# lcicek/Critic-VAE

Hardware: AMD Instinct MI355X
Metric: VAE train-step images/sec on 64x64x3 frames (higher is better)
Workload: dtype f32

## Files before the change

### critic-vae_amd/csrc/api.hip

```cpp
#include "common.h"
#include "../../include/cvae.h"
#include <stdarg.h>
#include <stdio.h>
#include <stdlib.h>
#include <string.h>
#include <cmath>
#include <string>
#include <vector>

static thread_local char g_err[512] = "";
void cvae_set_error(const char* fmt, ...) {
    va_list ap;
    va_start(ap, fmt);
    vsnprintf(g_err, sizeof(g_err), fmt, ap);
    va_end(ap);
}

static constexpr int PROBE_IDS = 32, PROBE_CAP = 128;
struct ProbeSlot { hipEvent_t e0[PROBE_CAP], e1[PROBE_CAP]; int n = 0; bool made = false; };
struct ProbeState { uint32_t mask = 0; ProbeSlot slot[PROBE_IDS]; };
static thread_local ProbeSlot* g_probe_cur = nullptr;
void cvae_probe_begin(hipStream_t st) {
    ProbeSlot* p = g_probe_cur;
    if (p && p->n < PROBE_CAP) (void)hipEventRecord(p->e0[p->n], st);
}
void cvae_probe_end(hipStream_t st) {
    ProbeSlot* p = g_probe_cur;
    if (p && p->n < PROBE_CAP) { (void)hipEventRecord(p->e1[p->n], st); p->n++; }
}

int cvae_num_cus() {
    constexpr int NCACHE = 64;
    static std::atomic<int> cached[NCACHE];
    int dev = 0;
    hipError_t e = hipGetDevice(&dev);
    if (e != hipSuccess) { cvae_set_error("cvae_num_cus: hipGetDevice failed (%s); assuming 256 compute units", hipGetErrorString(e)); return 256; }
    const bool cacheable = dev >= 0 && dev < NCACHE;
    int n = cacheable ? cached[dev].load(std::memory_order_relaxed) : 0;
    if (n > 0) return n;
    e = hipDeviceGetAttribute(&n, hipDeviceAttributeMultiprocessorCount, dev);
    if (e != hipSuccess || n <= 0) {
        cvae_set_error("cvae_num_cus: compute-unit query failed on device %d (%s); assuming 256", dev, hipGetErrorString(e));
        return 256;
    }
    if (cacheable) cached[dev].store(n, std::memory_order_relaxed);
    return n;
}

int persistent_grid(int wgs_per_cu, int num_items) {
    static const int maxwg = [] { const char* e = getenv("CVAE_PERSIST_MAXWG"); const int n = e ? atoi(e) : 0; return n > 0 ? n : 0; }();
    int G = wgs_per_cu * cvae_num_cus();
    if (maxwg > 0 && G > maxwg) G = maxwg;
    G -= G % 8;
    if (G < 8) G = 8;
    return G < num_items ? G : num_items;
}
extern "C" int32_t cvae_conv_route(int32_t precision, int32_t width, int32_t layer, int32_t dgrad, int64_t batch) {
    if ((width != 64 && width != 128) || layer < 0 || layer > 3 || precision < 0 || precision > 3 || batch < 1 || batch > 0x7fffffffLL) return CVAE_EINVAL;
    if (layer == 0 && (precision != 1 || dgrad != 0)) return CVAE_EINVAL;
    return conv_route(precision, layer, width, dgrad != 0, batch).family;
}

struct ParamEntry { std::string name; int64_t offset, numel; };

struct WsLayout {
    int64_t y[4], a[4], coef[4], bnpart[4];
    int64_t zcat, h, o[4];
    int64_t dout4, d_o[4], d_h, d_zcat, d_a[4], d_y[4];
    int64_t wc[3];
    int64_t xp;
    int64_t wpack;
    int64_t ms, scratch_w, scratch, total;
};

struct cvae_handle_s {
    cvae_config cfg;
    std::vector<ParamEntry> params;
    int64_t param_total;
    int K;
    int enc_w[4], enc_b[4], enc_g[4], enc_be[4], fc_w, fc_b, dec_w[5], dec_b[5], di_w, di_b;
    hipStream_t side = nullptr;
    hipEvent_t ev_ready[8] = {}, ev_side = nullptr;
    bool streams_ready = false;
    bool e1_two_pass = false;
    const void* xp_ws = nullptr;
    int xp_B = 0;
    bool fuse_e1 = true;
    ProbeState probe;
};

struct ProbeArm {
    ProbeArm(cvae_handle_s* h, int kind, int layer) {
        const int id = kind * 9 + layer;
        g_probe_cur = (h->probe.mask >> id) & 1u ? &h->probe.slot[id] : nullptr;
    }
    ~ProbeArm() { g_probe_cur = nullptr; }
};

static int ensure_streams(cvae_handle_s* h) {
    if (h->streams_ready) return 0;
    int lo = 0, hi = 0;
    hipError_t e = hipDeviceGetStreamPriorityRange(&lo, &hi);
    if (e == hipSuccess) e = hipStreamCreateWithPriority(&h->side, hipStreamNonBlocking, lo);
    for (int i = 0; i < 8 && e == hipSuccess; ++i) e = hipEventCreateWithFlags(&h->ev_ready[i], hipEventDisableTiming);
    if (e == hipSuccess) e = hipEventCreateWithFlags(&h->ev_side, hipEventDisableTiming);
    if (e != hipSuccess) { cvae_set_error("side stream setup failed: %s", hipGetErrorString(e)); return (int)e; }
    h->streams_ready = true;
    return 0;
}

static int layer_h(const cvae_handle_s* h, int layer) { return kLayers[layer].h * (h->cfg.width / 64); }

static WsLayout carve(const cvae_handle_s* h, int B) {
    WsLayout w{};
    const int W = h->cfg.width;
    int64_t off = 0;
    auto take = [&](int64_t n) { int64_t o = off; off += align_up(n, 64); return o; };
    const bool b16 = h->cfg.precision == 1;
    auto act = [&](int64_t elems) { return take(b16 ? (elems + 1) / 2 : elems); };
    for (int l = 0; l < 4; ++l) {
        const int64_t H = layer_h(h, l), C = kLayers[l].cout;
        w.y[l] = act(B * H * H * C);
        w.a[l] = act(B * (H / 2) * (H / 2) * C);
        w.coef[l] = take(C * 4);
        w.bnpart[l] = take((int64_t)2 * bn_num_tiles(l, W, B) * C);
        w.d_y[l] = (l == 0 && h->fuse_e1) ? -1 : act(B * H * H * C);
        w.d_a[l] = act(B * (H / 2) * (H / 2) * C);
    }
    w.zcat = take((int64_t)B * 33);
    w.d_zcat = take((int64_t)B * 33);
    w.h = act((int64_t)B * h->K);
    w.d_h = act((int64_t)B * h->K);
    for (int i = 0; i < 4; ++i) {
        const int64_t H = layer_h(h, 4 + i), C = kLayers[4 + i].cout;
        w.o[i] = act(B * H * H * C);
        w.d_o[i] = act(B * H * H * C);
    }
    w.dout4 = take(b16 ? 0 : (int64_t)B * 3 * W * W);
    for (int i = 0; i < 3; ++i) w.wc[i] = take(conv_up_wc_floats(5 + i));
    w.xp = take(b16 ? (int64_t)B * W * W * 2 : 0);
    w.wpack = take(h->cfg.precision != 0 ? conv_bf16_pack_floats(h->cfg.precision >= 2 ? 3 : 1) : 0);
    w.ms = take(msssim_ws_floats(W, B));
    int64_t sc = 0, scw = 0;
    auto mx = [&](int64_t v) { if (v > sc) sc = v; };
    for (int l = 1; l <= 4; ++l) { if (wgrad_ws_floats(l, W, B) > scw) scw = wgrad_ws_floats(l, W, B);
        if (h->cfg.precision == 1 && conv_bf16_supported(l, W) && wgrad_bf16_ws_floats(l, W, B) > scw) scw = wgrad_bf16_ws_floats(l, W, B);
        if (h->cfg.precision >= 2 && conv_bf16_supported(l, W) && wgrad_split_ws_floats(l, W, B) > scw) scw = wgrad_split_ws_floats(l, W, B);
        mx(conv_fwd_ws_floats(l, W, B)); mx(conv_dgrad_ws_floats(l, W, B)); }
    for (int l = 5; l <= 7; ++l) { if (conv_up_wgrad_ws_floats(l, W, B) > scw) scw = conv_up_wgrad_ws_floats(l, W, B); mx(conv_up_ws_floats(l, W, B)); }
    if (e1_wgrad_ws_floats(W, B) > scw) scw = e1_wgrad_ws_floats(W, B);
    w.scratch_w = take(scw);
    mx(scw + 36 * 128 * 64);
    mx(d4_bwd_ws_floats(W, B));
    for (int l = 0; l < 4; ++l) { mx(bn_bwd_ws_floats(l, W, B)); mx(bn_fwd_ws_floats(l, W)); }
    mx(fc_ws_floats(W, B));
    mx(colsum_ws_floats(0, 256));
    w.scratch = take(sc);
    w.total = off;
    return w;
}

static void add_param(cvae_handle_s* h, int* idx, const char* name, int64_t numel) {
    *idx = (int)h->params.size();
    h->params.push_back(ParamEntry{name, h->param_total, numel});
    h->param_total += align_up(numel, 64);
}

extern "C" {

const char* cvae_version(void) { return "critic-vae_amd 0.3 (gfx950; fp32 MFMA, bf16 MFMA with bf16 storage)"; }
const char* cvae_last_error(void) { return g_err; }

int cvae_create(const cvae_config* cfg, cvae_handle* out) {
    if (!cfg || !out) { cvae_set_error("cvae_create: null argument"); return CVAE_EINVAL; }
    if (cfg->width != 64 && cfg->width != 128) { cvae_set_error("cvae_create: width %d not supported (64 or 128)", cfg->width); return CVAE_EUNSUPPORTED; }
    if (cfg->precision < 0 || cfg->precision > 3) { cvae_set_error("cvae_create: precision %d not supported (0 = fp32, 1 = bf16 MFMA, 2 = fp32 emulated by 3-way bf16 splits)", cfg->precision); return CVAE_EUNSUPPORTED; }
    cvae_handle_s* h = new cvae_handle_s();
    h->cfg = *cfg;
    { const char* e = getenv("CVAE_FUSE_E1"); h->fuse_e1 = !(e && e[0] == '0'); }
    { const char* e = getenv("CVAE_E1_TWO_PASS"); h->e1_two_pass = cfg->precision == 1 && !(e && e[0] == '0'); }
    h->param_total = 0;
    h->K = 256 * (cfg->width / 16) * (cfg->width / 16);
    char nm[64];
    for (int l = 0; l < 4; ++l) {
        snprintf(nm, sizeof nm, "enc%d.w", l); add_param(h, &h->enc_w[l], nm, (int64_t)25 * kLayers[l].cin * kLayers[l].cout);
        snprintf(nm, sizeof nm, "enc%d.b", l); add_param(h, &h->enc_b[l], nm, kLayers[l].cout);
        snprintf(nm, sizeof nm, "enc%d.gamma", l); add_param(h, &h->enc_g[l], nm, kLayers[l].cout);
        snprintf(nm, sizeof nm, "enc%d.beta", l); add_param(h, &h->enc_be[l], nm, kLayers[l].cout);
    }
    add_param(h, &h->fc_w, "fc.w", (int64_t)h->K * 64);
    add_param(h, &h->fc_b, "fc.b", 64);
    for (int i = 0; i < 5; ++i) {
        snprintf(nm, sizeof nm, "dec%d.w", i); add_param(h, &h->dec_w[i], nm, (int64_t)25 * kLayers[4 + i].cin * kLayers[4 + i].cout);
        snprintf(nm, sizeof nm, "dec%d.b", i); add_param(h, &h->dec_b[i], nm, kLayers[4 + i].cout);
    }
    add_param(h, &h->di_w, "decin.w", (int64_t)33 * h->K);
    add_param(h, &h->di_b, "decin.b", h->K);
    *out = h;
    return CVAE_OK;
}

void cvae_destroy(cvae_handle h) {
    if (!h) return;
    if (h->streams_ready) {
        for (int i = 0; i < 8; ++i) (void)hipEventDestroy(h->ev_ready[i]);
        (void)hipEventDestroy(h->ev_side);
        (void)hipStreamDestroy(h->side);
    }
    delete h;
}

int64_t cvae_param_total(cvae_handle h) { return h->param_total; }
int32_t cvae_param_count(cvae_handle h) { return (int32_t)h->params.size(); }
// ... 452 lines not shown
```

### critic-vae_amd/csrc/common.h

```cpp
#pragma once
#include <hip/hip_runtime.h>
#include <stdint.h>
#include <stddef.h>
#include <atomic>

typedef float f32x16 __attribute__((ext_vector_type(16)));
typedef float f32x4 __attribute__((ext_vector_type(4)));
typedef __bf16 bf16x8 __attribute__((ext_vector_type(8)));

typedef __bf16 bf16x4 __attribute__((ext_vector_type(4)));

template <typename AT> struct Act;
template <> struct Act<float> {
    static constexpr bool BF16 = false;
    static __device__ __forceinline__ float ld(const float* p, size_t i) { return p[i]; }
    static __device__ __forceinline__ void st(float* p, size_t i, float v) { p[i] = v; }
    static __device__ __forceinline__ f32x4 ld4(const float* p, size_t i) { return *reinterpret_cast<const f32x4*>(p + i); }
    static __device__ __forceinline__ void st4(float* p, size_t i, f32x4 v) { *reinterpret_cast<f32x4*>(p + i) = v; }
};
template <> struct Act<__bf16> {
    static constexpr bool BF16 = true;
    static __device__ __forceinline__ float ld(const float* p, size_t i) { return (float)reinterpret_cast<const __bf16*>(p)[i]; }
    static __device__ __forceinline__ void st(float* p, size_t i, float v) { reinterpret_cast<__bf16*>(p)[i] = (__bf16)v; }
    static __device__ __forceinline__ f32x4 ld4(const float* p, size_t i) {
        const bf16x4 v = *reinterpret_cast<const bf16x4*>(reinterpret_cast<const __bf16*>(p) + i);
        return f32x4{(float)v[0], (float)v[1], (float)v[2], (float)v[3]};
    }
    static __device__ __forceinline__ void st4(float* p, size_t i, f32x4 v) {
        bf16x4 o;
        o[0] = (__bf16)v[0]; o[1] = (__bf16)v[1]; o[2] = (__bf16)v[2]; o[3] = (__bf16)v[3];
        *reinterpret_cast<bf16x4*>(reinterpret_cast<__bf16*>(p) + i) = o;
    }
    static __device__ __forceinline__ bf16x4 ld4raw(const float* p, size_t i) { return *reinterpret_cast<const bf16x4*>(reinterpret_cast<const __bf16*>(p) + i); }
    static __device__ __forceinline__ bf16x8 ld8(const float* p, size_t i) { return *reinterpret_cast<const bf16x8*>(reinterpret_cast<const __bf16*>(p) + i); }
    static __device__ __forceinline__ void st8(float* p, size_t i, bf16x8 v) { *reinterpret_cast<bf16x8*>(reinterpret_cast<__bf16*>(p) + i) = v; }
};

typedef short short4v __attribute__((ext_vector_type(4)));
typedef short short8v __attribute__((ext_vector_type(8)));
__device__ __forceinline__ bf16x8 tr_frag(const __bf16* p0, const __bf16* p1) {
    const short4v lo = __builtin_amdgcn_ds_read_tr16_b64_v4i16((__attribute__((address_space(3))) short4v*)p0);
    const short4v hi = __builtin_amdgcn_ds_read_tr16_b64_v4i16((__attribute__((address_space(3))) short4v*)p1);
    const short8v v = __builtin_shufflevector(lo, hi, 0, 1, 2, 3, 4, 5, 6, 7);
    return __builtin_bit_cast(bf16x8, v);
}

#define CVAE_LATENT 32
#define CVAE_ZCAT 33

struct LayerDesc { int cin, cout, h, up; };
static constexpr LayerDesc kLayers[9] = {
    {3, 32, 64, 0}, {32, 64, 32, 0}, {64, 128, 16, 0}, {128, 256, 8, 0},
    {256, 128, 4, 0}, {128, 64, 8, 1}, {64, 32, 16, 1}, {32, 32, 32, 1}, {32, 3, 64, 1}};

template <int H>
struct Tile {
    static constexpr int TW = H < 32 ? H : 32;
    static constexpr int TH = (128 / TW) < H ? (128 / TW) : H;
    static constexpr int IMGS = 128 / (TW * TH);
    static constexpr int HTW = TW + 4, HTH = TH + 4;
    static constexpr int HPI = HTW * HTH;
    static constexpr int HP = IMGS * HPI;
    static constexpr int PS = ((HP + 5) / 8) * 8 + 2;
    static constexpr int TILES_X = H / TW, TILES_Y = H / TH;
    static constexpr int TILES_PER_IMG = TILES_X * TILES_Y;
    static_assert(TW * TH * IMGS == 128, "tile must hold 128 pixels");
};

__host__ __device__ inline int cdiv(int a, int b) { return (a + b - 1) / b; }

__device__ __forceinline__ void vm_drained() { __builtin_amdgcn_s_waitcnt(0x0F70); }

__device__ __forceinline__ int xcd_tile(int x, int G) { return (G & 7) ? x : (x & 7) * (G >> 3) + (x >> 3); }
inline int64_t align_up(int64_t v, int64_t a) { return (v + a - 1) / a * a; }

__device__ __forceinline__ float wave_sum(float v) {
#pragma unroll
    for (int o = 32; o > 0; o >>= 1) v += __shfl_xor(v, o, 64);
    return v;
}
__device__ __forceinline__ double wave_sum_d(double v) {
#pragma unroll
    for (int o = 32; o > 0; o >>= 1) v += __shfl_xor(v, o, 64);
    return v;
}

__device__ __forceinline__ bool wg_arrive_last(unsigned* counter, unsigned total, unsigned* lds_word) {
    asm volatile("s_waitcnt vmcnt(0)" ::: "memory");
    __syncthreads();
    if (threadIdx.x == 0) {
        __builtin_amdgcn_fence(__ATOMIC_RELEASE, "agent");
        asm volatile("s_waitcnt vmcnt(0)" ::: "memory");
        const unsigned t = __hip_atomic_fetch_add(counter, 1u, __ATOMIC_RELAXED, __HIP_MEMORY_SCOPE_AGENT);
        const bool last = t == total - 1;
        if (last) {
            __hip_atomic_store(counter, 0u, __ATOMIC_RELAXED, __HIP_MEMORY_SCOPE_AGENT);
            __builtin_amdgcn_fence(__ATOMIC_ACQUIRE, "agent");
            asm volatile("s_waitcnt vmcnt(0)" ::: "memory");
        }
        *lds_word = last ? 1u : 0u;
    }
    __syncthreads();
    return *lds_word != 0u;
}

void cvae_probe_begin(hipStream_t st);
void cvae_probe_end(hipStream_t st);

void cvae_set_error(const char* fmt, ...);
#define CVAE_CHECK_LAUNCH()                                                        \
    do {                                                                           \
        hipError_t e_ = hipGetLastError();                                         \
        if (e_ != hipSuccess) {                                                    \
            cvae_set_error("%s:%d launch failed: %s", __FILE__, __LINE__,          \
                           hipGetErrorString(e_));                                 \
            return (int)e_;                                                        \
        }                                                                          \
    } while (0)

struct DeviceOnce { std::atomic<uint64_t> mask{0}; };
inline int cvae_grant_lds(DeviceOnce& once, const void* kernel, int bytes) {
    int dev = 0;
    hipError_t e = hipGetDevice(&dev);
    const uint64_t bit = 1ull << (dev & 63);
    if (e == hipSuccess && (once.mask.load(std::memory_order_acquire) & bit)) return 0;
    if (e == hipSuccess) e = hipFuncSetAttribute(kernel, hipFuncAttributeMaxDynamicSharedMemorySize, bytes);
    if (e != hipSuccess) { cvae_set_error("dynamic LDS opt-in (%d bytes) failed: %s", bytes, hipGetErrorString(e)); return (int)e; }
    once.mask.fetch_or(bit, std::memory_order_release);
    return 0;
}

int cvae_num_cus();
int persistent_grid(int wgs_per_cu, int num_items);

enum ConvFamily { CONV_PER_TILE = 0, CONV_PS = 1, CONV_BIG = 2, E1_PACKED_FRAME = 1 };
struct ConvRoute {
    ConvFamily family;
    int tilesPerPartial;
};
ConvRoute conv_route(int precision, int layer, int width, bool dgrad, int64_t B);

int launch_conv_fwd(int layer, int width, int B, const float* in, const float* w, const float* bias,
                    float* out, float* bnpart, float* ws, hipStream_t st);
int64_t conv_fwd_ws_floats(int layer, int width, int B);
int launch_conv_dgrad(int layer, int width, int B, const float* dout, const float* w,
                      const float* mask_src, float* din, float* ws, hipStream_t st);
int64_t conv_dgrad_ws_floats(int layer, int width, int B);
bool conv_bf16_supported(int layer, int width);
int64_t conv_bf16_pack_floats(int ns);
int launch_pack_w_bf16(const float* const w[4], float* packed, int ns, hipStream_t st);
int launch_conv_fwd_bf16(int layer, int width, int ns, int B, const float* in, const float* packed, const float* bias, float* out,
                         float* bnpart, float* ws, hipStream_t st, int* tilesPerPartial = nullptr);
int launch_conv_dgrad_bf16(int layer, int width, int ns, int B, const float* dout, const float* packed, float* din, float* ws, hipStream_t st);
int launch_pack_up_bf16(const float* const wc[3], float* packed, int ns, hipStream_t st);
int launch_conv_up_fwd_bf16(int layer, int width, int ns, int B, const float* in, const float* packed, const float* bias, float* out, hipStream_t st);
int launch_conv_up_dgrad_bf16(int layer, int width, int ns, int B, const float* dout, const float* packed, const float* aux, float* din, hipStream_t st);
int64_t wgrad_bf16_ws_floats(int layer, int width, int B);
int launch_conv_wgrad_bf16(int layer, int width, int B, const float* in, const float* dout, float* dw, float* dbias, float* ws, hipStream_t st);
bool conv_wgrad_split_supported(int products);
int64_t wgrad_split_ws_floats(int layer, int width, int B);
int launch_conv_wgrad_split(int layer, int width, int products, int B, const float* in, const float* dout, float* dw, float* dbias,
                            float* ws, hipStream_t st);
int launch_splitk_bias_relu(const float* slab, const float* bias, float* out, int64_t slice, int KS, int C, hipStream_t st, bool out_bf16 = false);
int64_t wgrad_ws_floats(int layer, int width, int B);
int launch_conv_wgrad(int layer, int width, int B, const float* in, const float* dout, float* dw,
                      float* dbias, float* ws, hipStream_t st);
int launch_reduce_slabs(const float* slab, float* dst, int64_t n, int S, int64_t stride, hipStream_t st,
                        float* mid = nullptr, bool out_bf16 = false);
int launch_colsum(const float* src, int64_t rows, int C, float* dst, float* ws, hipStream_t st);
int64_t colsum_ws_floats(int64_t rows, int C);
int64_t col_reduce_ws_floats(int W);
int launch_col_reduce_partial(const float* in, int R, int W, int64_t stride, float* ws, hipStream_t st,
                              const float** rows_out, int* R_out, int64_t* stride_out);
int launch_col_reduce(const float* in, int R, int W, int64_t stride, float* out, float* ws, hipStream_t st);
int launch_e1_fwd(int width, int B, const float* x, const float* w, const float* bias, float* y,
                  float* bnpart, hipStream_t st, bool bf16 = false, int pass = 0, const float* coef = nullptr, float* a1 = nullptr,
                  bool keep_y = true, float* xp = nullptr);
int launch_e1_wgrad(int width, int B, const float* x, const float* dy, float* dw, float* dbias, float* ws,
                    hipStream_t st, bool bf16 = false, const float* const* fuse = nullptr,
                    const float* xp = nullptr);
const float* bn_bwd_bcoef(int layer, int width, int B, const float* ws);
int64_t e1_wgrad_ws_floats(int width, int B);
int launch_d4_fwd(int width, int B, const float* in, const float* w, const float* bias, float* recon,
                  hipStream_t st, bool bf16io = false);
int64_t d4_bwd_ws_floats(int width, int B);
int launch_d4_bwd(int width, int B, const float* o3, const float* d_recon, const float* recon,
                  const float* w, float* dout, float* d_o3, float* dw, float* db, float* ws,
                  hipStream_t st, bool bf16io = false);
int64_t conv_up_wc_floats(int layer);
int launch_collapse_w(int layer, const float* w, float* wc, hipStream_t st);
int launch_collapse_w3(const float* const w[3], float* const wc[3], hipStream_t st);
int64_t conv_up_ws_floats(int layer, int width, int B);
int launch_conv_up_fwd(int layer, int width, int B, const float* in, const float* wc, const float* bias,
                       float* out, float* ws, hipStream_t st);
int launch_conv_up_dgrad(int layer, int width, int B, const float* dout, const float* wc, const float* aux,
                         float* din, float* ws, hipStream_t st);
int64_t conv_up_wgrad_ws_floats(int layer, int width, int B);
int launch_conv_up_wgrad(int layer, int width, int B, const float* in, const float* dout, float* dw,
                         float* dbias, float* ws, hipStream_t st, bool bf16 = false);
int launch_up_wgrad_bf16_main(int layer, int width, int B, const float* in, const float* dout, float* slab, int Smax, int* S_out, hipStream_t st);
int bn_num_tiles(int layer, int width, int B);
int launch_bn_fwd_finalize(int layer, int width, int B, const float* bnpart, const float* gamma,
                           const float* beta, float* run_mean, float* run_var, float* coef,
                           float* ws, int train, hipStream_t st, int tilesPerPartial = 1);
int64_t bn_fwd_ws_floats(int layer, int width);
int launch_bn_pool_act_fwd(int layer, int width, int B, const float* y, const float* coef, float* a,
                           hipStream_t st, bool bf16io = false);
int64_t bn_bwd_ws_floats(int layer, int width, int B);
int launch_bn_pool_act_bwd(int layer, int width, int B, const float* y, const float* a,
                           const float* da, const float* coef, const float* gamma, float* dy,
                           float* dgamma, float* dbeta, float* dbias, float* ws, hipStream_t st, bool bf16io = false);
int64_t fc_ws_floats(int width, int B);
int launch_fc_fwd(int width, int B, const float* flat, const float* wfc, const float* bfc,
                  const float* eps, const float* pred, float* mu, float* logvar, float* zcat,
                  float* ws, hipStream_t st, bool bf16io = false);
int launch_decin_fwd(int width, int B, const float* zcat, const float* wd, const float* bd, float* h,
                     hipStream_t st, bool bf16io = false);
int launch_decin_bwd(int width, int B, const float* zcat, const float* dh, const float* wd, float* dwd,
                     float* dbd, float* dzcat, float* ws, hipStream_t st, bool bf16io = false);
int launch_fc_bwd(int width, int B, const float* flat, const float* wfc, const float* dzcat,
                  const float* eps, const float* logvar, const float* dmu_loss,
                  const float* dlv_loss, float* dwfc, float* dbfc, float* dflat, float* ws,
                  hipStream_t st, bool bf16io = false);
int64_t msssim_ws_floats(int width, int B);
int launch_msssim(int width, int B, const float* img1, const float* img2, const float* mu,
                  const float* logvar, float* ws, float* scalars, float* d_img1, float* d_mu,
                  float* d_logvar, hipStream_t st);
int critic_param_count();
int launch_critic_fwd(int width, int B, const float* x, const float* critic_params, float* pred, hipStream_t st);
int launch_preprocess_u8(int width, int B, const uint8_t* u8, float* x, hipStream_t st);
int launch_diff_grey(int width, int B, const float* a, const float* b, float* diff, hipStream_t st);
int64_t crf_scratch_bytes(int width, int B);
int launch_dense_crf(int width, int B, const uint8_t* frames, const float* prob1, const struct cvae_crf_params& p,
                     uint8_t* labels, float* q1, void* scratch, hipStream_t st);
int launch_diff_normalize(int width, int B, const float* diff, double mean_max, double factor, int thr, const uint8_t* gt,
                          uint8_t* u8, uint8_t* mask, int64_t* counts, int64_t* hist, hipStream_t st);
int launch_mask_counts(int width, int B, const uint8_t* mask, const uint8_t* gt, int64_t* counts, hipStream_t st);
int launch_grads_bf16(const float* src_f32, void* bf16_buf, float* dst_f32, int64_t n, hipStream_t st);
int launch_adam(float* p, const float* g, float* m, float* v, int64_t n, int step, float lr, float b1,
                float b2, float eps, float gscale, hipStream_t st);
int launch_zero(float* p, int64_t n, hipStream_t st);
struct PadGaps { int64_t off[32]; int len[32]; int n; };
int launch_zero_gaps(float* grads, const PadGaps& gaps, hipStream_t st);
struct Scale3 { const float* g; const float* src[3]; float* dst[3]; int64_t n[3]; };
int launch_scale3(const Scale3& a, hipStream_t st);
```

### critic-vae_amd/csrc/conv_mfma.hip

```cpp
#include "common.h"
#include "conv_epilogue.h"


struct ConvRouteRow { int precision, layer, width; bool dgrad; ConvFamily family; int tilesPerPartial; };
static constexpr ConvRouteRow kConvRoutes[] = {
    {0, 1, 64, false, CONV_PS, 1}, {0, 2, 64, false, CONV_PS, 1}, {0, 3, 64, false, CONV_PS, 1},
    {0, 2, 64, true, CONV_PS, 1}, {0, 3, 64, true, CONV_PS, 1},
    {0, 1, 128, false, CONV_PS, 1}, {0, 2, 128, false, CONV_PS, 1}, {0, 2, 128, true, CONV_PS, 1},
    {1, 1, 64, false, CONV_BIG, 8}, {1, 2, 64, false, CONV_BIG, 4}, {1, 3, 64, false, CONV_BIG, 4},
    {1, 1, 64, true, CONV_BIG, 1}, {1, 2, 64, true, CONV_BIG, 1}, {1, 3, 64, true, CONV_BIG, 1},
    {1, 1, 128, false, CONV_BIG, 8}, {1, 2, 128, false, CONV_BIG, 4}, {1, 3, 128, false, CONV_BIG, 4},
    {1, 1, 128, true, CONV_BIG, 1}, {1, 2, 128, true, CONV_BIG, 1}, {1, 3, 128, true, CONV_BIG, 1},
    {1, 4, 128, false, CONV_PS, 1},
    {1, 0, 64, false, E1_PACKED_FRAME, 1}, {1, 0, 128, false, E1_PACKED_FRAME, 1},
};

ConvRoute conv_route(int precision, int layer, int width, bool dgrad, int64_t B) {
    static const bool per_tile_only = [] { const char* e = getenv("CVAE_CONV_PER_TILE"); return e && e[0] == '1'; }();
    const ConvRoute per_tile{CONV_PER_TILE, 1};
    for (const ConvRouteRow& r : kConvRoutes) {
        if (r.precision != precision || r.layer != layer || r.width != width || r.dgrad != dgrad) continue;
        if (layer == 0) {
            if (B * width * width * 8 + (2 * width + 2) * 8 >= (1ll << 31)) return per_tile;
            return {r.family, r.tilesPerPartial};
        }
        if (per_tile_only) return per_tile;
        const int64_t h = kLayers[layer].h * width / 64, c = kLayers[layer].cin > kLayers[layer].cout ? kLayers[layer].cin : kLayers[layer].cout;
        if (B * h * h * c * (precision == 1 ? 2 : 4) >= (1ll << 31)) return per_tile;
        return {r.family, r.tilesPerPartial};
    }
    return per_tile;
}


struct ConvArgs {
    const float* in;
    const float* w;
    const float* bias;
    const float* aux;
    float* out;
    float* bnpart;
    int B;
    int64_t sliceFloats;
};

template <int NT> struct KChunk { static constexpr int KC = NT == 32 ? 32 : 16, KCP = KC + 1; };


template <int KCH, int NCH, int H, bool DGRAD, int NT, int EPI, int KSPLIT>
__global__ __launch_bounds__(256) void conv5x5_mfma_kernel(ConvArgs a) {
    using T = Tile<H>;
    constexpr int NB = NT / 32;
    constexpr int KC = KChunk<NT>::KC, KCP = KChunk<NT>::KCP, QPP = KC / 4;
    constexpr int IN_FLOATS = KC * T::PS;
    constexpr int W_FLOATS = DGRAD ? 5 * NT * KCP : 5 * KC * NT;
    constexpr int EPI_FLOATS = (EPI == EPI_POOLSUM_MASK) ? 128 * (NT + 1) : 4 * 32 * 36;
    constexpr int SMEM = (IN_FLOATS + W_FLOATS) > EPI_FLOATS ? (IN_FLOATS + W_FLOATS) : EPI_FLOATS;
    __shared__ __attribute__((aligned(16))) float smem[SMEM];
    float* lds_in = smem;
    float* lds_w = smem + IN_FLOATS;

    const int tid = threadIdx.x, lane = tid & 63, wave = tid >> 6;
    const int li = lane & 31, lh = lane >> 5;
    const int mt = xcd_tile(blockIdx.x, gridDim.x), n0 = blockIdx.y * NT;
    const int tileInImg = mt % T::TILES_PER_IMG;
    const int img0 = (mt / T::TILES_PER_IMG) * T::IMGS;
    const int ty0 = (tileInImg / T::TILES_X) * T::TH, tx0 = (tileInImg % T::TILES_X) * T::TW;

    const int m = wave * 32 + li;
    const int pimg = m / (T::TH * T::TW), prem = m % (T::TH * T::TW);
    const int aBase = lh * T::PS + pimg * T::HPI + (prem / T::TW) * T::HTW + (prem % T::TW);
    const int bBase = DGRAD ? (li * KCP + lh) : (lh * NT + li);

    f32x16 acc[NB];
#pragma unroll
    for (int nb = 0; nb < NB; ++nb)
#pragma unroll
        for (int v = 0; v < 16; ++v) acc[nb][v] = 0.f;

    constexpr int WQ = 5 * KC * NT / 4;
    constexpr int WPT = (WQ + 255) / 256;
    f32x4 wreg[WPT];

    auto load_w = [&](int st) {
        const int cc = st / 5, r = st % 5;
#pragma unroll
        for (int i = 0; i < WPT; ++i) {
            const int q = tid + i * 256;
            if (WQ % 256 == 0 || q < WQ) {
                const float* src;
                if (!DGRAD) {
                    const int row = q / (NT / 4), c4 = q % (NT / 4);
                    const int s = row / KC, kc = row % KC;
                    src = a.w + (size_t)((r * 5 + s) * KCH + cc * KC + kc) * NCH + n0 + c4 * 4;
                } else {
                    const int c4 = q % QPP, rown = q / QPP;
                    const int n = rown % NT, s = rown / NT;
                    src = a.w + (size_t)((24 - (r * 5 + s)) * NCH + n0 + n) * KCH + cc * KC + c4 * 4;
                }
                wreg[i] = *reinterpret_cast<const f32x4*>(src);
            }
        }
    };
    auto store_w = [&]() {
#pragma unroll
        for (int i = 0; i < WPT; ++i) {
            const int q = tid + i * 256;
            if (WQ % 256 == 0 || q < WQ) {
                if (!DGRAD) {
                    *reinterpret_cast<f32x4*>(lds_w + q * 4) = wreg[i];
                } else {
                    const int c4 = q % QPP, rown = q / QPP;
                    float* d = lds_w + rown * KCP + c4 * 4;
                    d[0] = wreg[i].x; d[1] = wreg[i].y; d[2] = wreg[i].z; d[3] = wreg[i].w;
                }
            }
        }
    };
    constexpr int NQ = T::HP * (KC / 4), IPT = (NQ + 255) / 256;
    f32x4 ireg[IPT];
    auto load_input = [&](int cc) {
#pragma unroll
        for (int i = 0; i < IPT; ++i) {
            const int q = tid + i * 256;
            const int c4 = q % QPP, hp = q / QPP;
            const int img = hp / T::HPI, rem = hp - img * T::HPI;
            const int hy = rem / T::HTW, hx = rem - hy * T::HTW;
            const int gy = ty0 + hy - 2, gx = tx0 + hx - 2, ib = img0 + img;
            f32x4 v = {0.f, 0.f, 0.f, 0.f};
            if ((NQ % 256 == 0 || q < NQ) && (unsigned)gy < (unsigned)H && (unsigned)gx < (unsigned)H && ib < a.B)
                v = *reinterpret_cast<const f32x4*>(a.in + ((size_t)(ib * H + gy) * H + gx) * KCH + cc * KC + c4 * 4);
            ireg[i] = v;
        }
    };
    auto store_input = [&]() {
#pragma unroll
        for (int i = 0; i < IPT; ++i) {
            const int q = tid + i * 256;
            if (NQ % 256 == 0 || q < NQ) {
                float* d = lds_in + ((q % QPP) * 4) * T::PS + (q / QPP);
                d[0] = ireg[i].x; d[T::PS] = ireg[i].y; d[2 * T::PS] = ireg[i].z; d[3 * T::PS] = ireg[i].w;
            }
        }
    };

    static_assert((KCH / KC) % KSPLIT == 0, "split-K must divide the channel chunks");
    constexpr int NST = (KCH / KC) / KSPLIT * 5;
    const int st0 = blockIdx.z * NST, st1 = st0 + NST;
    [[maybe_unused]] float biasv[NB];
    if constexpr (KSPLIT == 1 && (EPI == EPI_BIAS_BNSTAT || EPI == EPI_BIAS_RELU)) load_bias<NT, EPI>(biasv, a.bias, n0);
    load_w(st0);
    load_input(st0 / 5);
    for (int st = st0; st < st1; ++st) {
        const int r = st % 5;
        __syncthreads();
        if (r == 0) store_input();
        store_w();
        if (r == 0 && st + 5 < st1) load_input(st / 5 + 1);
        if (st + 1 < st1) load_w(st + 1);
        __syncthreads();
        const float* ap = lds_in + aBase + r * T::HTW;
        __builtin_amdgcn_iglp_opt(0);
#pragma unroll
        for (int s = 0; s < 5; ++s) {
#pragma unroll
            for (int j = 0; j < KC / 2; ++j) {
                const float av = ap[(2 * j) * T::PS + s];
#pragma unroll
                for (int nb = 0; nb < NB; ++nb) {
                    const float bv = DGRAD ? lds_w[bBase + (s * NT + nb * 32) * KCP + 2 * j]
                                           : lds_w[bBase + (s * KC + 2 * j) * NT + nb * 32];
                    acc[nb] = __builtin_amdgcn_mfma_f32_32x32x2f32(av, bv, acc[nb], 0, 0, 0);
                }
            }
// ... 291 lines not shown
```

### critic-vae_amd/csrc/conv_wgrad.hip

```cpp
#include "common.h"

struct WgradArgs {
    const float* in;
    const float* dout;
    float* slab;
    int B;
    int numTiles;
    int tilesPerSplit;
};

template <int H, int W>
__device__ __forceinline__ void wgrad_body(f32x16 (&acc)[7], float& bsum, const float* lds_in, const float* lds_d, int li,
                                           int lh, int ty0, int tx0) {
    using T = Tile<H>;
    constexpr int CS = 32, R = T::IMGS * T::TH;
    for (int rho = 0; rho < R; ++rho) {
        const int img = rho / T::TH, ty = rho % T::TH, gy = ty0 + ty;
        const float* inrow = lds_in + ((img * T::HTH + ty) * T::HTW + lh) * CS + li;
        const float* drow = lds_d + (rho * T::TW + lh) * 32 + li;
        const bool extra = (rho & 3) == W && gy + 2 < H;
        constexpr int KKU = T::TW / 2 < 8 ? T::TW / 2 : 8;
#pragma unroll KKU
        for (int kk = 0; kk < T::TW / 2; ++kk) {
            const float bv = drow[(2 * kk) * 32];
            const int gx = tx0 + 2 * kk;
            if (W == 0) bsum += bv;
#pragma unroll
            for (int j = 0; j < 6; ++j) {
                const int tap = 4 * j + W, r = tap / 5, s = tap % 5;
                if ((unsigned)(gy + r - 2) < (unsigned)H && gx + s - 1 >= 0 && gx + s - 2 < H)
                    acc[j] = __builtin_amdgcn_mfma_f32_32x32x2f32(inrow[(r * T::HTW + s + 2 * kk) * CS], bv, acc[j], 0, 0, 0);
            }
            if (extra && gx + 2 < H)
                acc[6] = __builtin_amdgcn_mfma_f32_32x32x2f32(inrow[(4 * T::HTW + 4 + 2 * kk) * CS], bv, acc[6], 0, 0, 0);
        }
    }
}

template <int CIN, int COUT, int H, bool UP>
__global__ __launch_bounds__(256, 2) void conv5x5_wgrad_kernel(WgradArgs a) {
    using T = Tile<H>;
    constexpr int CS = 32;
    constexpr int IN_FLOATS = T::HP * CS;
    extern __shared__ __attribute__((aligned(16))) float smem[];
    float* lds_in = smem;
    float* lds_d = smem + IN_FLOATS;

    const int tid = threadIdx.x, lane = tid & 63, wave = tid >> 6;
    const int li = lane & 31, lh = lane >> 5;
    const int split = blockIdx.x, ci0 = blockIdx.y * 32, n0 = blockIdx.z * 32;
    constexpr int HS = UP ? H / 2 : H;

    f32x16 acc[7];
    float bsum = 0.f;
#pragma unroll
    for (int j = 0; j < 7; ++j)
#pragma unroll
        for (int v = 0; v < 16; ++v) acc[j][v] = 0.f;

    const int t0 = split * a.tilesPerSplit;
    int t1 = t0 + a.tilesPerSplit; if (t1 > a.numTiles) t1 = a.numTiles;

    constexpr int IQ = (T::HP * 8 + 255) / 256;
    f32x4 rin[IQ], rdo[4];
    auto fetch = [&](int mt) {
        const int tileInImg = mt % T::TILES_PER_IMG;
        const int img0 = (mt / T::TILES_PER_IMG) * T::IMGS;
        const int ty0 = (tileInImg / T::TILES_X) * T::TH, tx0 = (tileInImg % T::TILES_X) * T::TW;
#pragma unroll
        for (int i = 0; i < IQ; ++i) {
            const int q = tid + i * 256;
            const int c4 = q & 7, hp = q >> 3;
            const int img = hp / T::HPI, rem = hp % T::HPI;
            const int gy = ty0 + rem / T::HTW - 2, gx = tx0 + rem % T::HTW - 2, ib = img0 + img;
            f32x4 v = {0.f, 0.f, 0.f, 0.f};
            if (((T::HP * 8) % 256 == 0 || q < T::HP * 8) && (unsigned)gy < (unsigned)H && (unsigned)gx < (unsigned)H && ib < a.B) {
                const int sy = UP ? (gy >> 1) : gy, sx = UP ? (gx >> 1) : gx;
                v = *reinterpret_cast<const f32x4*>(a.in + ((size_t)(ib * HS + sy) * HS + sx) * CIN + ci0 + c4 * 4);
            }
            rin[i] = v;
        }
#pragma unroll
        for (int i = 0; i < 4; ++i) {
            const int q = tid + i * 256;
            const int c4 = q & 7, mm = q >> 3;
            const int im = mm / (T::TH * T::TW), rem = mm % (T::TH * T::TW);
            const int gy = ty0 + rem / T::TW, gx = tx0 + rem % T::TW, ib = img0 + im;
            f32x4 v = {0.f, 0.f, 0.f, 0.f};
            if (ib < a.B) v = *reinterpret_cast<const f32x4*>(a.dout + ((size_t)(ib * H + gy) * H + gx) * COUT + n0 + c4 * 4);
            rdo[i] = v;
        }
    };
    if (t0 < t1) fetch(t0);
    for (int mt = t0; mt < t1; ++mt) {
        const int tileInImg = mt % T::TILES_PER_IMG;
        const int ty0 = (tileInImg / T::TILES_X) * T::TH, tx0 = (tileInImg % T::TILES_X) * T::TW;
        __syncthreads();
#pragma unroll
        for (int i = 0; i < IQ; ++i) {
            const int q = tid + i * 256;
            if ((T::HP * 8) % 256 == 0 || q < T::HP * 8) *reinterpret_cast<f32x4*>(lds_in + (q >> 3) * CS + (q & 7) * 4) = rin[i];
        }
#pragma unroll
        for (int i = 0; i < 4; ++i) {
            const int q = tid + i * 256;
            *reinterpret_cast<f32x4*>(lds_d + (q >> 3) * 32 + (q & 7) * 4) = rdo[i];
        }
        __syncthreads();
        if (mt + 1 < t1) fetch(mt + 1);
        switch (wave) {
            case 0: wgrad_body<H, 0>(acc, bsum, lds_in, lds_d, li, lh, ty0, tx0); break;
            case 1: wgrad_body<H, 1>(acc, bsum, lds_in, lds_d, li, lh, ty0, tx0); break;
            case 2: wgrad_body<H, 2>(acc, bsum, lds_in, lds_d, li, lh, ty0, tx0); break;
            default: wgrad_body<H, 3>(acc, bsum, lds_in, lds_d, li, lh, ty0, tx0); break;
        }
    }

    float* out = a.slab + (size_t)split * (25 * CIN * COUT + COUT);
    if (wave == 0 && blockIdx.y == 0) {
        bsum += __shfl_xor(bsum, 32, 64);
        if (lh == 0) out[(size_t)25 * CIN * COUT + n0 + li] = bsum;
    }
#pragma unroll
    for (int j = 0; j < 6; ++j)
#pragma unroll
        for (int v = 0; v < 16; ++v) {
            const int ci = ci0 + (v & 3) + 8 * (v >> 2) + 4 * lh;
            out[((size_t)(4 * j + wave) * CIN + ci) * COUT + n0 + li] = acc[j][v];
        }
    __syncthreads();
    if (wave > 0) {
#pragma unroll
        for (int v = 0; v < 16; ++v) smem[((wave - 1) * 16 + v) * 64 + lane] = acc[6][v];
    }
    __syncthreads();
    if (wave == 0) {
#pragma unroll
        for (int v = 0; v < 16; ++v) {
            const float x = ((acc[6][v] + smem[v * 64 + lane]) + smem[(16 + v) * 64 + lane]) + smem[(32 + v) * 64 + lane];
            const int ci = ci0 + (v & 3) + 8 * (v >> 2) + 4 * lh;
            out[((size_t)24 * CIN + ci) * COUT + n0 + li] = x;
        }
    }
}

template <typename AT>
__global__ __launch_bounds__(256) void reduce_slabs_kernel(const float* __restrict__ slab, float* __restrict__ dst,
                                                           int64_t n, int S, int64_t stride, int perChunk) {
    const int64_t i = ((int64_t)blockIdx.x * 256 + threadIdx.x) * 4;
    if (i >= n) return;
    const int s0 = blockIdx.y * perChunk;
    int s1 = s0 + perChunk; if (s1 > S) s1 = S;
    float4 acc = make_float4(0.f, 0.f, 0.f, 0.f);
#pragma unroll 8
    for (int s = s0; s < s1; ++s) {
        const float4 v = *reinterpret_cast<const float4*>(slab + (size_t)s * stride + i);
        acc.x += v.x; acc.y += v.y; acc.z += v.z; acc.w += v.w;
    }
    Act<AT>::st4(dst, (size_t)blockIdx.y * n + i, f32x4{acc.x, acc.y, acc.z, acc.w});
}

__global__ __launch_bounds__(256) void reduce_slabs_wide_kernel(const float* __restrict__ slab, float* __restrict__ dst,
                                                                int64_t n4, int S, int64_t stride) {
    __shared__ f32x4 red[16][16];
    const int oi = threadIdx.x & 15, g = threadIdx.x >> 4;
    const int64_t o = (int64_t)blockIdx.x * 16 + oi;
    f32x4 acc = {0.f, 0.f, 0.f, 0.f};
    if (o < n4) {
#pragma unroll 4
        for (int r = g; r < S; r += 16) acc += *reinterpret_cast<const f32x4*>(slab + (size_t)r * stride + o * 4);
    }
    red[g][oi] = acc;
    __syncthreads();
    if (g == 0 && o < n4) {
#pragma unroll
        for (int k = 1; k < 16; ++k) acc += red[k][oi];
        *reinterpret_cast<f32x4*>(dst + o * 4) = acc;
    }
}

int launch_reduce_slabs(const float* slab, float* dst, int64_t n, int S, int64_t stride, hipStream_t st, float* mid, bool out_bf16) {
    (void)mid;
    if (out_bf16) {
        const unsigned gx = (unsigned)((n / 4 + 255) / 256);
        hipLaunchKernelGGL(reduce_slabs_kernel<__bf16>, dim3(gx, 1), dim3(256), 0, st, slab, dst, n, S, stride, S);
        CVAE_CHECK_LAUNCH();
        return 0;
    }
    if (S > 32) {
        const int64_t n4 = n / 4;
        hipLaunchKernelGGL(reduce_slabs_wide_kernel, dim3((unsigned)((n4 + 15) / 16)), dim3(256), 0, st, slab, dst, n4, S, stride);
        CVAE_CHECK_LAUNCH();
        return 0;
    }
    const unsigned gx = (unsigned)((n / 4 + 255) / 256);
    hipLaunchKernelGGL(reduce_slabs_kernel<float>, dim3(gx, 1), dim3(256), 0, st, slab, dst, n, S, stride, S);
    CVAE_CHECK_LAUNCH();
    return 0;
}

template <int H>
static int wgrad_splits(int B, int blocksPerSplit, int* tilesPerSplit) {
    using T = Tile<H>;
    const int numTiles = cdiv(B, T::IMGS) * T::TILES_PER_IMG;
    int S = cdiv(512, blocksPerSplit);
    if (S > numTiles) S = numTiles;
    if (S < 1) S = 1;
    const int tps = cdiv(numTiles, S);
    S = cdiv(numTiles, tps);
    *tilesPerSplit = tps;
    return S;
}

template <int CIN, int COUT, int H, bool UP>
static int run_wgrad(int B, const float* in, const float* dout, float* dw, float* dbias, float* ws, hipStream_t st,
                     int64_t* ws_need) {
    using T = Tile<H>;
    int tps;
    const int bps = (CIN / 32) * (COUT / 32);
    const int S = wgrad_splits<H>(B, bps, &tps);
    const int64_t n = (int64_t)25 * CIN * COUT, row = n + COUT;
    if (ws_need) { *ws_need = (int64_t)(S + 16) * row; return 0; }
    WgradArgs a{in, dout, ws, B, cdiv(B, T::IMGS) * T::TILES_PER_IMG, tps};
    constexpr int SMEM = (T::HP * 32 + 128 * 32) * 4;
    auto kern = conv5x5_wgrad_kernel<CIN, COUT, H, UP>;
    static DeviceOnce once;
    { int rc = cvae_grant_lds(once, reinterpret_cast<const void*>(kern), SMEM); if (rc) return rc; }
    cvae_probe_begin(st);
    hipLaunchKernelGGL(kern, dim3(S, CIN / 32, COUT / 32), dim3(256), SMEM, st, a);
    cvae_probe_end(st);
    CVAE_CHECK_LAUNCH();
    float* mid = ws + (size_t)S * row;
    if (dbias == dw + n)
        return launch_reduce_slabs(ws, dw, row, S, row, st, mid);
    int rc = launch_reduce_slabs(ws, dw, n, S, row, st, mid);
    if (rc || !dbias) return rc;
    return launch_reduce_slabs(ws + n, dbias, COUT, S, row, st, nullptr);
}

static int dispatch_wgrad(int layer, int width, int B, const float* in, const float* dout, float* dw, float* dbias,
                          float* ws, hipStream_t st, int64_t* need) {
    if (width == 64) {
        switch (layer) {
            case 1: return run_wgrad<32, 64, 32, false>(B, in, dout, dw, dbias, ws, st, need);
            case 2: return run_wgrad<64, 128, 16, false>(B, in, dout, dw, dbias, ws, st, need);
            case 3: return run_wgrad<128, 256, 8, false>(B, in, dout, dw, dbias, ws, st, need);
            case 4: return run_wgrad<256, 128, 4, false>(B, in, dout, dw, dbias, ws, st, need);
        }
    }
    if (width == 128) {
        switch (layer) {
            case 1: return run_wgrad<32, 64, 64, false>(B, in, dout, dw, dbias, ws, st, need);
            case 2: return run_wgrad<64, 128, 32, false>(B, in, dout, dw, dbias, ws, st, need);
            case 3: return run_wgrad<128, 256, 16, false>(B, in, dout, dw, dbias, ws, st, need);
            case 4: return run_wgrad<256, 128, 8, false>(B, in, dout, dw, dbias, ws, st, need);
        }
    }
    cvae_set_error("conv_wgrad: unsupported layer %d at width %d", layer, width);
    return -2;
}

int64_t wgrad_ws_floats(int layer, int width, int B) {
    int64_t need = 0;
    if (dispatch_wgrad(layer, width, B, nullptr, nullptr, nullptr, nullptr, nullptr, nullptr, &need) != 0) return 0;
    return need;
}

int launch_conv_wgrad(int layer, int width, int B, const float* in, const float* dout, float* dw, float* dbias,
                      float* ws, hipStream_t st) {
    return dispatch_wgrad(layer, width, B, in, dout, dw, dbias, ws, st, nullptr);
}

static constexpr int CS_BLOCKS = 128;

__global__ __launch_bounds__(256) void colsum_stage1(const float* __restrict__ src, int64_t rows, int C,
                                                     float* __restrict__ part) {
    __shared__ float red[256];
    const int c = threadIdx.x % C, rl = threadIdx.x / C, RL = 256 / C;
    const int64_t per = (rows + gridDim.x - 1) / gridDim.x;
    const int64_t r0 = blockIdx.x * per;
    int64_t r1 = r0 + per; if (r1 > rows) r1 = rows;
    float acc = 0.f;
    for (int64_t r = r0 + rl; r < r1; r += RL) acc += src[r * C + c];
    red[threadIdx.x] = acc;
    __syncthreads();
    if (rl == 0) {
        for (int k = 1; k < RL; ++k) acc += red[k * C + c];
        part[(size_t)blockIdx.x * C + c] = acc;
    }
}

int64_t colsum_ws_floats(int64_t rows, int C) { (void)rows; return (int64_t)CS_BLOCKS * C + col_reduce_ws_floats(C); }

int launch_colsum(const float* src, int64_t rows, int C, float* dst, float* ws, hipStream_t st) {
    if (C > 256 || 256 % C != 0) { cvae_set_error("colsum: C=%d unsupported", C); return -2; }
    int nblk = CS_BLOCKS;
    if (nblk > rows) nblk = (int)rows;
    hipLaunchKernelGGL(colsum_stage1, dim3(nblk), dim3(256), 0, st, src, rows, C, ws);
    CVAE_CHECK_LAUNCH();
    return launch_col_reduce(ws, nblk, C, C, dst, ws + (size_t)CS_BLOCKS * C, st);
}
```

Baseline: 88230.

## Add persistent double-buffered fp32 wgrad kernel routed per layer

Adds a persistent 512-thread fp32 weight-gradient kernel. Each workgroup loops over (split, channel-block) items and covers 64 output channels. Input and gradient tiles are prefetched into registers and staged into double-buffered LDS, so global loads overlap the second half of the row loop. A new 'pass=2' route table picks which layers and widths use it; other cases keep the original per-tile kernel. This aims to cut launch and tail overhead and hide load latency, at the cost of one workgroup per CU and higher register and LDS pressure.

```diff
diff --git a/critic-vae_amd/csrc/api.hip b/critic-vae_amd/csrc/api.hip
--- a/critic-vae_amd/csrc/api.hip
+++ b/critic-vae_amd/csrc/api.hip
@@ -56,9 +56,10 @@
     return G < num_items ? G : num_items;
 }
 extern "C" int32_t cvae_conv_route(int32_t precision, int32_t width, int32_t layer, int32_t dgrad, int64_t batch) {
-    if ((width != 64 && width != 128) || layer < 0 || layer > 3 || precision < 0 || precision > 3 || batch < 1 || batch > 0x7fffffffLL) return CVAE_EINVAL;
+    if ((width != 64 && width != 128) || layer < 0 || layer > 4 || precision < 0 || precision > 3 || batch < 1 || batch > 0x7fffffffLL) return CVAE_EINVAL;
     if (layer == 0 && (precision != 1 || dgrad != 0)) return CVAE_EINVAL;
-    return conv_route(precision, layer, width, dgrad != 0, batch).family;
+    if (layer == 4 && dgrad != 2) return CVAE_EINVAL;
+    return conv_route(precision, layer, width, dgrad == 2 ? 2 : dgrad != 0, batch).family;
 }
 
 struct ParamEntry { std::string name; int64_t offset, numel; };
diff --git a/critic-vae_amd/csrc/common.h b/critic-vae_amd/csrc/common.h
--- a/critic-vae_amd/csrc/common.h
+++ b/critic-vae_amd/csrc/common.h
@@ -138,7 +138,7 @@
     ConvFamily family;
     int tilesPerPartial;
 };
-ConvRoute conv_route(int precision, int layer, int width, bool dgrad, int64_t B);
+ConvRoute conv_route(int precision, int layer, int width, int pass, int64_t B);
 
 int launch_conv_fwd(int layer, int width, int B, const float* in, const float* w, const float* bias,
                     float* out, float* bnpart, float* ws, hipStream_t st);
diff --git a/critic-vae_amd/csrc/conv_mfma.hip b/critic-vae_amd/csrc/conv_mfma.hip
--- a/critic-vae_amd/csrc/conv_mfma.hip
+++ b/critic-vae_amd/csrc/conv_mfma.hip
@@ -2,11 +2,13 @@
 #include "conv_epilogue.h"
 
 
-struct ConvRouteRow { int precision, layer, width; bool dgrad; ConvFamily family; int tilesPerPartial; };
+struct ConvRouteRow { int precision, layer, width, pass; ConvFamily family; int tilesPerPartial; };
 static constexpr ConvRouteRow kConvRoutes[] = {
     {0, 1, 64, false, CONV_PS, 1}, {0, 2, 64, false, CONV_PS, 1}, {0, 3, 64, false, CONV_PS, 1},
     {0, 2, 64, true, CONV_PS, 1}, {0, 3, 64, true, CONV_PS, 1},
     {0, 1, 128, false, CONV_PS, 1}, {0, 2, 128, false, CONV_PS, 1}, {0, 2, 128, true, CONV_PS, 1},
+    {0, 1, 64, 2, CONV_PS, 1}, {0, 2, 64, 2, CONV_PS, 1}, {0, 4, 64, 2, CONV_PS, 1},
+    {0, 1, 128, 2, CONV_PS, 1}, {0, 2, 128, 2, CONV_PS, 1}, {0, 3, 128, 2, CONV_PS, 1},
     {1, 1, 64, false, CONV_BIG, 8}, {1, 2, 64, false, CONV_BIG, 4}, {1, 3, 64, false, CONV_BIG, 4},
     {1, 1, 64, true, CONV_BIG, 1}, {1, 2, 64, true, CONV_BIG, 1}, {1, 3, 64, true, CONV_BIG, 1},
     {1, 1, 128, false, CONV_BIG, 8}, {1, 2, 128, false, CONV_BIG, 4}, {1, 3, 128, false, CONV_BIG, 4},
@@ -15,11 +17,11 @@
     {1, 0, 64, false, E1_PACKED_FRAME, 1}, {1, 0, 128, false, E1_PACKED_FRAME, 1},
 };
 
-ConvRoute conv_route(int precision, int layer, int width, bool dgrad, int64_t B) {
+ConvRoute conv_route(int precision, int layer, int width, int pass, int64_t B) {
     static const bool per_tile_only = [] { const char* e = getenv("CVAE_CONV_PER_TILE"); return e && e[0] == '1'; }();
     const ConvRoute per_tile{CONV_PER_TILE, 1};
     for (const ConvRouteRow& r : kConvRoutes) {
-        if (r.precision != precision || r.layer != layer || r.width != width || r.dgrad != dgrad) continue;
+        if (r.precision != precision || r.layer != layer || r.width != width || r.pass != pass) continue;
         if (layer == 0) {
             if (B * width * width * 8 + (2 * width + 2) * 8 >= (1ll << 31)) return per_tile;
             return {r.family, r.tilesPerPartial};
diff --git a/critic-vae_amd/csrc/conv_wgrad.hip b/critic-vae_amd/csrc/conv_wgrad.hip
--- a/critic-vae_amd/csrc/conv_wgrad.hip
+++ b/critic-vae_amd/csrc/conv_wgrad.hip
@@ -9,20 +9,20 @@
     int tilesPerSplit;
 };
 
-template <int H, int W>
+template <int H, int W, int DS = 32, int RHO0 = 0, int RHO1 = Tile<H>::IMGS * Tile<H>::TH, int KU = 8>
 __device__ __forceinline__ void wgrad_body(f32x16 (&acc)[7], float& bsum, const float* lds_in, const float* lds_d, int li,
                                            int lh, int ty0, int tx0) {
     using T = Tile<H>;
-    constexpr int CS = 32, R = T::IMGS * T::TH;
-    for (int rho = 0; rho < R; ++rho) {
+    constexpr int CS = 32;
+    for (int rho = RHO0; rho < RHO1; ++rho) {
         const int img = rho / T::TH, ty = rho % T::TH, gy = ty0 + ty;
         const float* inrow = lds_in + ((img * T::HTH + ty) * T::HTW + lh) * CS + li;
-        const float* drow = lds_d + (rho * T::TW + lh) * 32 + li;
+        const float* drow = lds_d + (rho * T::TW + lh) * DS + li;
         const bool extra = (rho & 3) == W && gy + 2 < H;
-        constexpr int KKU = T::TW / 2 < 8 ? T::TW / 2 : 8;
+        constexpr int KKU = T::TW / 2 < KU ? T::TW / 2 : KU;
 #pragma unroll KKU
         for (int kk = 0; kk < T::TW / 2; ++kk) {
-            const float bv = drow[(2 * kk) * 32];
+            const float bv = drow[(2 * kk) * DS];
             const int gx = tx0 + 2 * kk;
             if (W == 0) bsum += bv;
 #pragma unroll
@@ -140,6 +140,163 @@
             const float x = ((acc[6][v] + smem[v * 64 + lane]) + smem[(16 + v) * 64 + lane]) + smem[(32 + v) * 64 + lane];
             const int ci = ci0 + (v & 3) + 8 * (v >> 2) + 4 * lh;
             out[((size_t)24 * CIN + ci) * COUT + n0 + li] = x;
+        }
+    }
+}
+
+struct WgradPsArgs {
+    const float* in;
+    const float* dout;
+    float* slab;
+    int B;
+    int numTiles;
+    int tilesPerSplit;
+    int items;
+};
+
+template <int CIN, int COUT, int H>
+struct WgradPs {
+    using T = Tile<H>;
+    static constexpr int NB = (CIN / 32) * (COUT / 64);
+    static constexpr int STAGE = T::HP * 32 + 128 * 64;
+    static constexpr bool DB = 2 * STAGE * 4 <= 160 * 1024;
+    static constexpr int SMEM = (DB ? 2 : 1) * STAGE * 4;
+    static_assert(SMEM <= 160 * 1024 && 6 * 16 * 64 <= STAGE, "LDS");
+};
+
+template <int A, int B> struct RowRange { static constexpr int first = A, second = B; };
+
+template <int CIN, int COUT, int H>
+__global__ __launch_bounds__(512, 1) void conv5x5_wgrad_ps_kernel(WgradPsArgs a) {
+    using T = Tile<H>;
+    using P = WgradPs<CIN, COUT, H>;
+    constexpr int CS = 32, R = T::IMGS * T::TH, NCB = COUT / 64;
+    constexpr int KU = H == 8 ? 2 : 8;
+    extern __shared__ __attribute__((aligned(16))) float smem[];
+    const int tid = threadIdx.x, lane = tid & 63, wave = tid >> 6, tg = wave & 3, cb = wave >> 2;
+    const int li = lane & 31, lh = lane >> 5;
+
+    constexpr int IQ = (T::HP * 8 + 511) / 512;
+    f32x4 rin[IQ], rdo[4];
+    int ci0 = 0, n0 = 0;
+    auto fetch = [&](int mt) {
+        const int tileInImg = mt % T::TILES_PER_IMG;
+        const int img0 = (mt / T::TILES_PER_IMG) * T::IMGS;
+        const int ty0 = (tileInImg / T::TILES_X) * T::TH, tx0 = (tileInImg % T::TILES_X) * T::TW;
+#pragma unroll
+        for (int i = 0; i < IQ; ++i) {
+            const int q = tid + i * 512;
+            const int c4 = q & 7, hp = q >> 3;
+            const int img = hp / T::HPI, rem = hp % T::HPI;
+            const int gy = ty0 + rem / T::HTW - 2, gx = tx0 + rem % T::HTW - 2, ib = img0 + img;
+            f32x4 v = {0.f, 0.f, 0.f, 0.f};
+            if (((T::HP * 8) % 512 == 0 || q < T::HP * 8) && (unsigned)gy < (unsigned)H && (unsigned)gx < (unsigned)H && ib < a.B)
+                v = *reinterpret_cast<const f32x4*>(a.in + ((size_t)(ib * H + gy) * H + gx) * CIN + ci0 + c4 * 4);
+            rin[i] = v;
+        }
+#pragma unroll
+        for (int i = 0; i < 4; ++i) {
+            const int q = tid + i * 512;
+            const int c4 = q & 15, mm = q >> 4;
+            const int im = mm / (T::TH * T::TW), rem = mm % (T::TH * T::TW);
+            const int gy = ty0 + rem / T::TW, gx = tx0 + rem % T::TW, ib = img0 + im;
+            f32x4 v = {0.f, 0.f, 0.f, 0.f};
+            if (ib < a.B) v = *reinterpret_cast<const f32x4*>(a.dout + ((size_t)(ib * H + gy) * H + gx) * COUT + n0 + c4 * 4);
+            rdo[i] = v;
+        }
+    };
+    auto stage = [&](float* buf) {
+#pragma unroll
+        for (int i = 0; i < IQ; ++i) {
+            const int q = tid + i * 512;
+            if ((T::HP * 8) % 512 == 0 || q < T::HP * 8) *reinterpret_cast<f32x4*>(buf + (q >> 3) * CS + (q & 7) * 4) = rin[i];
+        }
+#pragma unroll
+        for (int i = 0; i < 4; ++i) {
+            const int q = tid + i * 512;
+            *reinterpret_cast<f32x4*>(buf + T::HP * CS + (q >> 4) * 64 + (q & 15) * 4) = rdo[i];
+        }
+    };
+    auto body = [&](auto rows, f32x16 (&acc)[7], float& bsum, const float* buf, int ty0, int tx0) {
+        constexpr int R0 = decltype(rows)::first, R1 = decltype(rows)::second;
+        const float* ld = buf + T::HP * CS + cb * 32;
+        switch (tg) {
+            case 0: wgrad_body<H, 0, 64, R0, R1, KU>(acc, bsum, buf, ld, li, lh, ty0, tx0); break;
+            case 1: wgrad_body<H, 1, 64, R0, R1, KU>(acc, bsum, buf, ld, li, lh, ty0, tx0); break;
+            case 2: wgrad_body<H, 2, 64, R0, R1, KU>(acc, bsum, buf, ld, li, lh, ty0, tx0); break;
+            default: wgrad_body<H, 3, 64, R0, R1, KU>(acc, bsum, buf, ld, li, lh, ty0, tx0); break;
+        }
+    };
+
+    for (int item = xcd_tile(blockIdx.x, gridDim.x); item < a.items; item += gridDim.x) {
+        const int split = item / P::NB, blk = item % P::NB;
+        ci0 = (blk / NCB) * 32;
+        n0 = (blk % NCB) * 64;
+        const int t0 = split * a.tilesPerSplit;
+        int t1 = t0 + a.tilesPerSplit; if (t1 > a.numTiles) t1 = a.numTiles;
+
+        f32x16 acc[7];
+        float bsum = 0.f;
+#pragma unroll
+        for (int j = 0; j < 7; ++j)
+#pragma unroll
+            for (int v = 0; v < 16; ++v) acc[j][v] = 0.f;
+
+        __syncthreads();
+        fetch(t0);
+        if constexpr (P::DB) {
+            stage(smem);
+            if (t0 + 1 < t1) fetch(t0 + 1);
+        }
+        for (int mt = t0; mt < t1; ++mt) {
+            const int tileInImg = mt % T::TILES_PER_IMG;
+            const int ty0 = (tileInImg / T::TILES_X) * T::TH, tx0 = (tileInImg % T::TILES_X) * T::TW;
+            if constexpr (P::DB) {
+                float* buf = smem + ((mt - t0) & 1) * P::STAGE;
+                float* nbuf = smem + ((mt - t0 + 1) & 1) * P::STAGE;
+                __syncthreads();
+                body(RowRange<0, R / 2>{}, acc, bsum, buf, ty0, tx0);
+                if (mt + 1 < t1) {
+                    stage(nbuf);
+                    if (mt + 2 < t1) fetch(mt + 2);
+                }
+                body(RowRange<R / 2, R>{}, acc, bsum, buf, ty0, tx0);
+            } else {
+                if (mt > t0) __syncthreads();
+                stage(smem);
+                __syncthreads();
+                if (mt + 1 < t1) fetch(mt + 1);
+                body(RowRange<0, R>{}, acc, bsum, smem, ty0, tx0);
+            }
+        }
+
+        float* out = a.slab + (size_t)split * (25 * CIN * COUT + COUT);
+        const int nc = n0 + cb * 32;
+        if (tg == 0 && ci0 == 0) {
+            bsum += __shfl_xor(bsum, 32, 64);
+            if (lh == 0) out[(size_t)25 * CIN * COUT + nc + li] = bsum;
+        }
+#pragma unroll
+        for (int j = 0; j < 6; ++j)
+#pragma unroll
+            for (int v = 0; v < 16; ++v) {
+                const int ci = ci0 + (v & 3) + 8 * (v >> 2) + 4 * lh;
+                out[((size_t)(4 * j + tg) * CIN + ci) * COUT + nc + li] = acc[j][v];
+            }
+        __syncthreads();
+        if (tg > 0) {
+#pragma unroll
+            for (int v = 0; v < 16; ++v) smem[((cb * 3 + tg - 1) * 16 + v) * 64 + lane] = acc[6][v];
+        }
+        __syncthreads();
+        if (tg == 0) {
+            const float* red = smem + cb * 3 * 16 * 64;
+#pragma unroll
+            for (int v = 0; v < 16; ++v) {
+                const float x = ((acc[6][v] + red[v * 64 + lane]) + red[(16 + v) * 64 + lane]) + red[(32 + v) * 64 + lane];
+                const int ci = ci0 + (v & 3) + 8 * (v >> 2) + 4 * lh;
+                out[((size_t)24 * CIN + ci) * COUT + nc + li] = x;
+            }
         }
     }
 }
@@ -214,22 +371,39 @@
 
 template <int CIN, int COUT, int H, bool UP>
 static int run_wgrad(int B, const float* in, const float* dout, float* dw, float* dbias, float* ws, hipStream_t st,
-                     int64_t* ws_need) {
+                     int64_t* ws_need, bool persistent) {
     using T = Tile<H>;
     int tps;
     const int bps = (CIN / 32) * (COUT / 32);
     const int S = wgrad_splits<H>(B, bps, &tps);
     const int64_t n = (int64_t)25 * CIN * COUT, row = n + COUT;
     if (ws_need) { *ws_need = (int64_t)(S + 16) * row; return 0; }
-    WgradArgs a{in, dout, ws, B, cdiv(B, T::IMGS) * T::TILES_PER_IMG, tps};
-    constexpr int SMEM = (T::HP * 32 + 128 * 32) * 4;
-    auto kern = conv5x5_wgrad_kernel<CIN, COUT, H, UP>;
-    static DeviceOnce once;
-    { int rc = cvae_grant_lds(once, reinterpret_cast<const void*>(kern), SMEM); if (rc) return rc; }
-    cvae_probe_begin(st);
-    hipLaunchKernelGGL(kern, dim3(S, CIN / 32, COUT / 32), dim3(256), SMEM, st, a);
-    cvae_probe_end(st);
-    CVAE_CHECK_LAUNCH();
+    const int numTiles = cdiv(B, T::IMGS) * T::TILES_PER_IMG;
+    persistent = persistent && !UP && COUT % 64 == 0;
+    if constexpr (!UP && COUT % 64 == 0) {
+        if (persistent) {
+            using P = WgradPs<CIN, COUT, H>;
+            WgradPsArgs a{in, dout, ws, B, numTiles, tps, S * P::NB};
+            auto kern = conv5x5_wgrad_ps_kernel<CIN, COUT, H>;
+            static DeviceOnce once;
+            { int rc = cvae_grant_lds(once, reinterpret_cast<const void*>(kern), P::SMEM); if (rc) return rc; }
+            cvae_probe_begin(st);
+            hipLaunchKernelGGL(kern, dim3(persistent_grid(1, a.items)), dim3(512), P::SMEM, st, a);
+            cvae_probe_end(st);
+            CVAE_CHECK_LAUNCH();
+        }
+    }
+    if (!persistent) {
+        WgradArgs a{in, dout, ws, B, numTiles, tps};
+        constexpr int SMEM = (T::HP * 32 + 128 * 32) * 4;
+        auto kern = conv5x5_wgrad_kernel<CIN, COUT, H, UP>;
+        static DeviceOnce once;
+        { int rc = cvae_grant_lds(once, reinterpret_cast<const void*>(kern), SMEM); if (rc) return rc; }
+        cvae_probe_begin(st);
+        hipLaunchKernelGGL(kern, dim3(S, CIN / 32, COUT / 32), dim3(256), SMEM, st, a);
+        cvae_probe_end(st);
+        CVAE_CHECK_LAUNCH();
+    }
     float* mid = ws + (size_t)S * row;
     if (dbias == dw + n)
         return launch_reduce_slabs(ws, dw, row, S, row, st, mid);
@@ -240,20 +414,21 @@
 
 static int dispatch_wgrad(int layer, int width, int B, const float* in, const float* dout, float* dw, float* dbias,
                           float* ws, hipStream_t st, int64_t* need) {
+    const bool ps = !need && conv_route(0, layer, width, 2, B).family == CONV_PS;
     if (width == 64) {
         switch (layer) {
-            case 1: return run_wgrad<32, 64, 32, false>(B, in, dout, dw, dbias, ws, st, need);
-            case 2: return run_wgrad<64, 128, 16, false>(B, in, dout, dw, dbias, ws, st, need);
-            case 3: return run_wgrad<128, 256, 8, false>(B, in, dout, dw, dbias, ws, st, need);
-            case 4: return run_wgrad<256, 128, 4, false>(B, in, dout, dw, dbias, ws, st, need);
+            case 1: return run_wgrad<32, 64, 32, false>(B, in, dout, dw, dbias, ws, st, need, ps);
+            case 2: return run_wgrad<64, 128, 16, false>(B, in, dout, dw, dbias, ws, st, need, ps);
+            case 3: return run_wgrad<128, 256, 8, false>(B, in, dout, dw, dbias, ws, st, need, ps);
+            case 4: return run_wgrad<256, 128, 4, false>(B, in, dout, dw, dbias, ws, st, need, ps);
         }
     }
     if (width == 128) {
         switch (layer) {
-            case 1: return run_wgrad<32, 64, 64, false>(B, in, dout, dw, dbias, ws, st, need);
-            case 2: return run_wgrad<64, 128, 32, false>(B, in, dout, dw, dbias, ws, st, need);
-            case 3: return run_wgrad<128, 256, 16, false>(B, in, dout, dw, dbias, ws, st, need);
-            case 4: return run_wgrad<256, 128, 8, false>(B, in, dout, dw, dbias, ws, st, need);
+            case 1: return run_wgrad<32, 64, 64, false>(B, in, dout, dw, dbias, ws, st, need, ps);
+            case 2: return run_wgrad<64, 128, 32, false>(B, in, dout, dw, dbias, ws, st, need, ps);
+            case 3: return run_wgrad<128, 256, 16, false>(B, in, dout, dw, dbias, ws, st, need, ps);
+            case 4: return run_wgrad<256, 128, 8, false>(B, in, dout, dw, dbias, ws, st, need, ps);
         }
     }
     cvae_set_error("conv_wgrad: unsupported layer %d at width %d", layer, width);
```

After: 88930 (median of 6 runs). About the same (+0.8%).
